# a-rtemis99/hpc_suffix_array

Hardware: AMD Instinct MI355X
Metric: suffixes sorted/sec + ms/doubling-round, 1 GiB input at 1/2/4/8 MI355X (higher is better)
Workload: dtype u32

## Files before the change

### hpc_suffix_array_amd/_native.py

```python
from __future__ import annotations

import ctypes
import os
import subprocess

PKG_DIR = os.path.dirname(os.path.abspath(__file__))
LIB_PATH = os.path.join(PKG_DIR, "lib", "libsa_hip.so")
LIB_PATH = os.environ.get("SA_LIB_PATH", LIB_PATH)
CSRC = os.path.join(PKG_DIR, "csrc")

SA_MAX_ROUNDS = 64
KERNEL_KINDS = ["init", "hist_first", "hist_keys", "scan", "scatter_first", "scatter_keys",
                "heads", "heads_scan", "rerank", "seg_count", "seg_scan", "seg_write", "alphabet", "pack",
                "sort_u", "windows", "local_sort", "pivot_keys", "pivot_count", "pivot_write"]
SCHEDULE_PACKED = 0
SCHEDULE_REFERENCE = 1
ROUND1_AUTO = 0
ROUND1_LSD = 1
ROUND1_BUCKETED = 2
SA_K_COUNT = len(KERNEL_KINDS)
FIND_AUTO = 0
FIND_LANE = 1
FIND_WAVE = 2
FIND_LANE_MAX = 3584
# ... 41 lines not shown
EXT_SYMBOLS = ["sa_context_create", "sa_context_destroy", "sa_context_set_debug", "sa_workspace_bytes", "sa_build_device",
               "sa_build_ex", "sa_check_device", "sa_check", "sa_lcp_device", "sa_lcp", "sa_generate_text_device",
               "sa_alphabet_device", "sa_pack_keys_device", "sa_sort_pairs_device", "sa_scatter_u64_device",
               "sa_gather_u64_device", "sa_running_max_i64_device", "sa_inclusive_sum_i64_device",
               "sa_count_below_u64_device", "sa_select_u8_device",
               "sa_find_device", "sa_find", "sa_find_ex",
               "sa_match_device", "sa_matching_stats_device", "sa_match", "sa_matching_stats",
               "sa_bwt_device", "sa_bwt", "sa_inverse_device", "sa_inverse",
               "sa_locate_device", "sa_locate",
               "sa_mems_device", "sa_mems",
               "sa_lpf_device", "sa_lpf", "sa_lz77_device", "sa_lz77",
               "sa_repeats_device", "sa_repeats",
               "sa_lf_device", "sa_ibwt_device", "sa_lf", "sa_ibwt", "sa_ibwt_ex",
               "sa_fm_index_bytes", "sa_fm_build_device", "sa_fm_count_device", "sa_fm_locate_device",
               "sa_fm_build", "sa_fm_count", "sa_fm_locate",
               "sa_doc_array_device", "sa_doc_of_device", "sa_doc_frequency_device", "sa_doc_list_device",
               "sa_doc_array", "sa_doc_of", "sa_doc_frequency", "sa_doc_list",
               "sa_lce_index_bytes", "sa_lce_build_device", "sa_lcp_min_device", "sa_lce_device",
               "sa_substr_compare_device", "sa_lcp_min", "sa_lce", "sa_substr_compare",
               "sa_dist_begin", "sa_dist_cuts", "sa_dist_plan_cuts", "sa_dist_reserve", "sa_dist_release", "sa_dist_round1", "sa_dist_req_count", "sa_dist_req_fill",
               "sa_dist_answer", "sa_dist_refine",
               "sa_last_error", "sa_host_syncs", "sa_device_count", "sa_version", "sa_struct_size"]


class SAError(RuntimeError):
    """A libsa_hip entry point returned an error code."""


DEBUG_FLAGS = {"no_cmp": 0x1, "no_pk8": 0x2, "no_pad": 0x4, "pad_overflow": 0x8, "no_fast32": 0x10,
               "no_pivot": 0x20, "perm_always": 0x40, "no_xq": 0x80, "xq_overflow": 0x100,
               "no_tied": 0x200, "no_key1_round": 0x400, "no_eonly": 0x800,
               "eonly": 0x1000, "fast32_small": 0x2000, "no_round2_fused": 0x4000,
               "ls_one_wg": 0x8000, "no_alpha_sample": 0x10000, "alpha_sample_small": 0x20000,
               "bb17": 0x40000, "bb18": 0x80000}


def debug_bits(names) -> int:
    bits = 0
    for x in names or ():
        if x not in DEBUG_FLAGS:
            raise ValueError(f"unknown debug flag {x!r} (one of {sorted(DEBUG_FLAGS)})")
        bits |= DEBUG_FLAGS[x]
    return bits


class SaOpts(ctypes.Structure):
    _fields_ = [("profile", ctypes.c_int32), ("schedule", ctypes.c_int32), ("init_chars", ctypes.c_int32),
                ("radix", ctypes.c_int32), ("round1", ctypes.c_int32), ("debug", ctypes.c_uint32),
                ("span_extra", ctypes.c_int32), ("tune", ctypes.c_int32)]


class SaStats(ctypes.Structure):
    _fields_ = [
        ("rounds", ctypes.c_int32),
        ("n_kinds", ctypes.c_int32),
        ("total_ms", ctypes.c_double),
        ("h2d_ms", ctypes.c_double),
        ("d2h_ms", ctypes.c_double),
        ("round_ms", ctypes.c_double * SA_MAX_ROUNDS),
        ("distinct", ctypes.c_uint64 * SA_MAX_ROUNDS),
        ("passes", ctypes.c_int32 * SA_MAX_ROUNDS),
        ("sorted_n", ctypes.c_uint64 * SA_MAX_ROUNDS),
        ("prefix_len", ctypes.c_uint64 * SA_MAX_ROUNDS),
        ("schedule", ctypes.c_int32),
        ("init_chars", ctypes.c_int32),
        ("sigma", ctypes.c_int32),
        ("sparse_ranks", ctypes.c_int32),
# ... 290 lines not shown
```

### hpc_suffix_array_amd/csrc/sa_bucket.h

```cpp
#pragma once
#include <type_traits>

#include "sa_kernels.h"

namespace sa {

#ifndef SA_BS_BLOCK
#define SA_BS_BLOCK 512
#endif
constexpr int kBsBlock = SA_BS_BLOCK;
#ifndef SA_BS_ITEMS
#define SA_BS_ITEMS 18
#endif
constexpr int kBsItems = SA_BS_ITEMS;
constexpr int kBsCap = kBsBlock * kBsItems;
constexpr uint32_t kWinStride = 1024;
#ifndef SA_BS_WPC
#define SA_BS_WPC 2
#endif
constexpr uint32_t kBsWpc = SA_BS_WPC;
#ifndef SA_BS_GRID
#define SA_BS_GRID (1u << 22)
#endif
constexpr uint32_t kBsGrid = SA_BS_GRID;
constexpr uint64_t kBucketMinN = 1ull << 20;
constexpr uint32_t kLoBits = 8;
constexpr uint32_t kLoRadix = 1u << kLoBits;

__device__ __forceinline__ uint32_t bucket_of(uint64_t key1, uint32_t rb, uint64_t cmul, uint32_t bsh) {
    return (uint32_t)(((key1 >> rb) * cmul) >> bsh);
}

__device__ __forceinline__ uint32_t bucket_dmin(uint32_t b, uint64_t cmul, uint32_t bsh) {
    const uint64_t d0 = ((uint64_t)b << bsh) / cmul;
    return (uint32_t)((((d0 * cmul) >> bsh) == b) ? d0 : d0 + 1);
}
// ... 1271 lines not shown
                    }
                }
            }
        }
        probe.mark(5);
        store_window<BLOCK, ITEMS>(s_w, a, m, ib, mn, keys_out, sa_out, so.ksh);
        __syncthreads();
        probe.mark(6);
    }
    probe.flush(words);
    flush_totals(words, th, tu, tg);
}

template <int ITEMS>
__device__ __forceinline__ uint32_t slot0() {
    uint32_t t = threadIdx.x;
    asm volatile("" : "+v"(t));
    return (t / kWave) * (kWave * ITEMS) + (t & (kWave - 1));
}

constexpr uint32_t kSlotBits = kBsCap > (1 << 14) ? 15 : 14;
constexpr uint32_t kSlotMask = (1u << kSlotBits) - 1u;
constexpr uint32_t kLowMax = 32 - kSlotBits;
static_assert(kBsCap <= (1 << kSlotBits), "load slots in kSlotBits");
constexpr int kHdrWord = 14;
constexpr int kTicketWord = 15;

__global__ __launch_bounds__(kBlock) void k_window_split(const uint32_t* __restrict__ list,
                                                         const uint32_t* __restrict__ ws, BucketRel br,
                                                         uint32_t* __restrict__ words, uint4* __restrict__ hdr,
                                                         uint32_t* __restrict__ retry, uint32_t fast,
                                                         const uint32_t* __restrict__ pc = nullptr,
                                                         const uint32_t* __restrict__ pn = nullptr, uint32_t nb = 0,
                                                         uint32_t* __restrict__ hx = nullptr, uint32_t crows = 0) {
    const uint32_t nlist = words[7];
    const uint32_t lane = lane_id();
    for (uint64_t q0 = (uint64_t)blockIdx.x * kBlock; q0 < nlist; q0 += (uint64_t)gridDim.x * kBlock) {
        const uint64_t q = q0 + threadIdx.x;
        uint32_t j = 0, b0 = 0;
        bool one = false;
        const bool ok = q < nlist;
        if (ok) {
            j = list[q];
            b0 = br.wb[j];
            one = fast && br.wb[j + 1] - b0 == 1u;
            if (one && hx) {
                uint32_t nr = 0;
                for (uint32_t k = 0; k < kXq; ++k) {
                    const uint32_t c = pn[(uint64_t)k * nb + b0];
                    if (!crows && c && c < kWave) one = false;
                    nr += (c + kWave - 1) / kWave;
                }
                if (crows && nr > crows) one = false;
            }
        }
        const uint64_t m1 = __ballot(ok && one), m2 = __ballot(ok && !one);
        uint32_t base1 = 0, base2 = 0;
        if (lane == 0) {
            if (m1) base1 = atomicAdd(&words[kHdrWord], (uint32_t)__popcll(m1));
            if (m2) base2 = atomicAdd(&words[kRetryWord], (uint32_t)__popcll(m2));
        }
        base1 = (uint32_t)__shfl((int)base1, 0, kWave);
        base2 = (uint32_t)__shfl((int)base2, 0, kWave);
        if (ok && one) {
            const uint32_t a = ws[j];
            const uint32_t qi = base1 + (uint32_t)__popcll(m1 & lanemask_lt());
            hdr[qi] = make_uint4(j, a, ws[j + 1] - a, br.bdmin[b0]);
            if (hx) {
                uint32_t P = 0;
                for (uint32_t k = 0; k < kXq; ++k) {
                    const uint32_t c = pc[(uint64_t)k * nb + b0];
                    hx[(uint64_t)qi * 16 + k] = c - P;
                    if (k) hx[(uint64_t)qi * 16 + kXq - 1 + k] = P;
                    P += pn[(uint64_t)k * nb + b0];
                }
            }
        } else if (ok) {
            retry[base2 + (uint32_t)__popcll(m2 & lanemask_lt())] = j;
        }
    }
}

__global__ __launch_bounds__(kBlock) void k_window_gather(const uint32_t* __restrict__ list,
                                                          const uint32_t* __restrict__ words,
                                                          const uint32_t* __restrict__ ws,
                                                          const uint32_t* __restrict__ wb,
                                                          const uint32_t* __restrict__ pc,
                                                          const uint32_t* __restrict__ pn, uint32_t nb,
                                                          const uint64_t* __restrict__ in,
                                                          uint64_t* __restrict__ out) {
    const uint32_t nlist = words[kRetryWord];
    for (uint32_t qi = blockIdx.x; qi < nlist; qi += gridDim.x) {
        const uint32_t j = list[qi];
        uint64_t dst = ws[j];
        for (uint32_t b = wb[j]; b < wb[j + 1]; ++b) {
            for (uint32_t k = 0; k < kXq; ++k) {
                const uint32_t c = pn[(uint64_t)k * nb + b];
                const uint64_t src = pc[(uint64_t)k * nb + b];
                for (uint32_t t = threadIdx.x; t < c; t += kBlock) out[dst + t] = in[src + t];
                dst += c;
            }
        }
    }
}

template <int N, int LSV = 0>
__device__ __forceinline__ bool sort_sub_words(uint32_t* __restrict__ s_k, const uint32_t* __restrict__ s_x,
// ... 38 lines not shown
        const uint32_t x = s_k[k];
        uint32_t y = k;
        while (y > lo && s_k[y - 1] > x) {
            s_k[y] = s_k[y - 1];
            --y;
        }
        s_k[y] = x;
    }
    uint32_t pr = ~0u, cur = s_k[lo] >> kSlotBits;
    for (uint32_t k = lo; k < hi; ++k) {
        const uint32_t nx = k + 1 < hi ? (s_k[k + 1] >> kSlotBits) : ~0u;
        const bool eqp = k > lo && pr == cur, eqn = k + 1 < hi && nx == cur;
        nu += (eqp || eqn) ? 1u : 0u;
        ng += (!eqp && eqn) ? 1u : 0u;
        pr = cur;
        cur = nx;
    }
}

template <int ITEMS, int I0 = 0, int I1 = ITEMS>
__device__ __forceinline__ void load_items(const uint64_t* __restrict__ w_in, uint64_t a, uint32_t m,
                                           uint64_t (&x)[ITEMS]) {
    const uint32_t l0 = slot0<ITEMS>();
#pragma unroll
    for (int i = I0; i < I1; ++i) {
        const uint32_t le = l0 + i * kWave;
        x[i] = w_in[a + (le < m ? le : m - 1)];
    }
}

struct XqWin {
    const uint32_t* __restrict__ hx = nullptr;
    const uint32_t* __restrict__ rows = nullptr;
};

__device__ __forceinline__ uint32_t xq_offset(const uint32_t* __restrict__ hx, uint32_t le) {
    uint32_t off = hx[0];
#pragma unroll
    for (int k = 1; k < (int)kXq; ++k) off = hx[kXq - 1 + k] <= le ? hx[k] : off;
    return off;
}

template <int ITEMS, int I0 = 0, int I1 = ITEMS>
__device__ __forceinline__ void load_items_cr(const uint64_t* __restrict__ w_in, const uint32_t (&rv)[3],
                                              uint64_t (&x)[ITEMS]) {
    const uint32_t lane = lane_id();
#pragma unroll
    for (int i = I0; i < I1; ++i) {
        const uint32_t base = (uint32_t)__builtin_amdgcn_readlane((int)rv[0], i);
        x[i] = (w_in + base)[lane];
    }
}

template <int ITEMS, int ROWS>
__device__ __forceinline__ void load_rows_xq(const uint32_t* __restrict__ rows, uint32_t (&rv)[3]) {
    const uint32_t lane = lane_id();
    const uint32_t w = (uint32_t)__builtin_amdgcn_readfirstlane((int)(threadIdx.x / kWave));
    const uint32_t r = w * ITEMS + (lane < (uint32_t)ITEMS ? lane : 0u);
#pragma unroll
    for (int t = 0; t < 3; ++t) rv[t] = rows[t * ROWS + r];
}

template <int ITEMS, int I0 = 0, int I1 = ITEMS>
__device__ __forceinline__ void load_items_xq(const uint64_t* __restrict__ w_in, const uint32_t (&rv)[3], uint32_t m,
                                              uint64_t (&x)[ITEMS]) {
    const uint32_t l0 = slot0<ITEMS>();
    const uint32_t lane = lane_id();
    const uint32_t last = m - 1;
#pragma unroll
    for (int i = I0; i < I1; ++i) {
        const uint32_t le = l0 + i * kWave;
        const uint32_t lc = le < m ? le : last;
        const uint32_t da = (uint32_t)__builtin_amdgcn_readlane((int)rv[0], i);
        const uint32_t db = (uint32_t)__builtin_amdgcn_readlane((int)rv[1], i);
        const uint32_t sp = (uint32_t)__builtin_amdgcn_readlane((int)rv[2], i);
        x[i] = w_in[(uint32_t)((lane < sp ? da : db) + lc)];
    }
}

template <bool CR>
__global__ __launch_bounds__(kBlock) void k_window_rows(const uint32_t* __restrict__ words, const uint4* __restrict__ hdr,
                                                        const uint32_t* __restrict__ hx, uint32_t nrows,
                                                        uint32_t* __restrict__ rows) {
    const uint32_t nh = words[kHdrWord];
    const uint32_t lane = lane_id();
    for (uint64_t q = (uint64_t)blockIdx.x * kWaves + wave_id(); q < nh; q += (uint64_t)gridDim.x * kWaves) {
        const uint32_t m = hdr[q].z;
        uint32_t hv[16];
#pragma unroll
        for (int k = 0; k < 16; ++k) hv[k] = hx[q * 16 + k];
        if constexpr (CR) {
            uint32_t st[kXq], cn[kXq], nfull = 0;
#pragma unroll
            for (int k = 0; k < (int)kXq; ++k) {
                const uint32_t p0 = k ? hv[kXq - 1 + k] : 0u, p1 = k + 1 < (int)kXq ? hv[kXq + k] : m;
                st[k] = hv[k] + p0;
                cn[k] = p1 - p0;
                nfull += cn[k] / kWave;
            }
            for (uint32_t r = lane; r < nrows; r += kWave) {
                uint32_t base = st[0], cnt = 0, rf = 0, rp = nfull;
#pragma unroll
                for (int k = 0; k < (int)kXq; ++k) {
                    const uint32_t nf = cn[k] / kWave, rem = cn[k] % kWave;
                    if (r >= rf && r < rf + nf) {
                        base = st[k] + kWave * (r - rf);
                        cnt = kWave;
                    }
                    if (rem && r == rp) {
                        base = st[k] + kWave * nf;
                        cnt = rem;
                    }
                    rf += nf;
                    rp += rem ? 1u : 0u;
                }
                uint32_t* const e = rows + q * 3 * nrows + r;
                e[0] = base;
                e[nrows] = cnt;
            }
            continue;
        }
        for (uint32_t r = lane; r < nrows; r += kWave) {
            const uint32_t lo = std::min(r * kWave, m - 1), hi = std::min(r * kWave + (kWave - 1), m - 1);
            uint32_t split = kWave;
#pragma unroll
            for (int k = kXq - 1; k >= 1; --k) {
                const uint32_t pk = hv[kXq - 1 + k];
                if (pk > lo && pk <= hi) split = pk - r * kWave;
            }
            uint32_t* const e = rows + q * 3 * nrows + r;
            e[0] = xq_offset(hv, lo);
            e[nrows] = xq_offset(hv, hi);
            e[2 * nrows] = split;
        }
    }
}

#ifndef SA_LS_WFULL
#define SA_LS_WFULL 1
#endif
#ifndef SA_LS_CLAIMS
#define SA_LS_CLAIMS 1
#endif
#ifndef SA_LS_HRANK
#define SA_LS_HRANK 1
#endif
#ifndef SA_LS_HRANK_PF
#define SA_LS_HRANK_PF 3
#endif
#if SA_LS_HRANK_PF == 0
#define SA_LS_PF_TABLE {0, 0, 18, 18, 18}
#elif SA_LS_HRANK_PF == 1
#define SA_LS_PF_TABLE {18, 18, 18, 18, 18}
#elif SA_LS_HRANK_PF == 3
#define SA_LS_PF_TABLE {6, 6, 12, 18, 18}
#elif SA_LS_HRANK_PF == 5
#define SA_LS_PF_TABLE {0, 0, 6, 12, 18}
#elif SA_LS_HRANK_PF == 6
#define SA_LS_PF_TABLE {3, 6, 9, 15, 18}
#endif
constexpr int kLsPfHr[5] = SA_LS_PF_TABLE;
constexpr int kLsPfOld[5] = {0, 0, 18, 18, 18};
template <int P>
using pf_point = std::integral_constant<int, P>;
template <int BLOCK, int ITEMS, class Probe = NoProbe, bool XQ = false, int LSV = 0, bool CR = false>
__global__ __launch_bounds__(BLOCK, 4) void k_bucket_sort(const uint64_t* __restrict__ keys_in,
                                                       const uint4* __restrict__ hdr, uint32_t rb, uint32_t bits,
                                                       uint32_t ib, uint32_t* __restrict__ words,
                                                       uint64_t* __restrict__ keys_out, uint32_t* __restrict__ sa_out,
                                                       uint32_t* __restrict__ retry, SegOut so, XqWin xw = XqWin{}) {
    constexpr int WAVES = BLOCK / kWave;
    constexpr int CAP = BLOCK * ITEMS;
    static_assert(CAP <= (1 << kSlotBits), "load slots");
    __shared__ uint32_t s_lds[kSubBuckets / 2 + CAP + ((LSV & 1) ? kNet : 0) + CAP];
    uint32_t* const s_cnt = s_lds;
    uint32_t* const s_k = s_lds + kSubBuckets / 2;
    uint32_t* const s_x = s_k + CAP + ((LSV & 1) ? kNet : 0);
    __shared__ uint32_t s_tmp[WAVES];
    __shared__ uint32_t s_cm[WAVES];
    __shared__ uint32_t s_ug[WAVES];
    __shared__ uint32_t s_q[2];
    __shared__ unsigned long long s_tot[3];
    constexpr int WPT = kSubBuckets / 2 / BLOCK;
    static_assert(WPT * 2 == 4 && WPT * 2 * BLOCK == kSubBuckets, "four sub-buckets per thread");
    constexpr int ROWS = WAVES * ITEMS;

    const uint32_t wave = wave_id(), lane = lane_id();
    const uint32_t dg = threadIdx.x;
    const uint32_t nwin = words[kHdrWord];
    const uint32_t low_bits = bits - kSubBits;
    const uint32_t dsh = ib + low_bits;
    const uint32_t lmask = (1u << low_bits) - 1u;
    const uint64_t imask = (1ull << ib) - 1ull;
    auto end_of = [&](uint32_t sb) -> uint32_t { return ((s_cnt[sb >> 1] >> (16 * (sb & 1))) & 0xFFFFu) >> 2; };
    static_assert(4 * CAP < (1 << 16), "byte counts in 16-bit halves");
    auto cnt_word = [&](uint32_t y) -> uint32_t* {
        return reinterpret_cast<uint32_t*>(reinterpret_cast<char*>(s_cnt) + ((y << 1) & 0xFFCu));
    };
    auto half_inc = [](uint32_t y) -> uint32_t {
        uint32_t r;
        asm("v_lshlrev_b32_e64 %0, %1, 4" : "=v"(r) : "v"(y << 4));
        return r;
    };
    constexpr bool HR = SA_LS_HRANK != 0;
    typedef uint16_t __attribute__((may_alias)) half_t;
    Probe probe;
    if (threadIdx.x == 0) {
        s_q[0] = atomicAdd(&words[kTicketWord], 1u);
        if constexpr (HR) s_q[1] = atomicAdd(&words[kTicketWord], 1u);
        s_tot[0] = s_tot[1] = s_tot[2] = 0;
    }
    if constexpr (HR)
        for (int i = threadIdx.x; i < kSubBuckets / 2; i += BLOCK) s_cnt[i] = 0;
    __syncthreads();
    uint32_t q = (uint32_t)__builtin_amdgcn_readfirstlane((int)s_q[0]);
    if (q >= nwin) return;
    uint4 h = hdr[q];
    uint64_t w[ITEMS];
    uint32_t rv[3] = {0u, 0u, 0u};
    if constexpr (XQ) {
        load_rows_xq<ITEMS, ROWS>(xw.rows + (uint64_t)q * 3 * ROWS, rv);
        if constexpr (CR) load_items_cr<ITEMS>(keys_in, rv, w);
        else load_items_xq<ITEMS>(keys_in, rv, h.z, w);
    } else {
        load_items<ITEMS>(keys_in, h.y, h.z, w);
    }
    uint32_t qn = 0;
    bool more = false;
    uint4 hn = make_uint4(0u, 0u, 1u, 0u);
    uint32_t rwn[3] = {0u, 0u, 0u};
    auto next_window = [&](uint32_t ticket, uint32_t cur, uint32_t& qx, bool& mx, uint4& hx,
                           uint32_t (&rx)[3]) __attribute__((always_inline)) {
        qx = (uint32_t)__builtin_amdgcn_readfirstlane((int)ticket);
        mx = qx < nwin;
        hx = make_uint4(0u, 0u, 1u, 0u);
        if (mx) hx = hdr[qx];
        if constexpr (XQ) load_rows_xq<ITEMS, ROWS>(xw.rows + (uint64_t)(mx ? qx : cur) * 3 * ROWS, rx);
    };
    if constexpr (HR) next_window(s_q[1], q, qn, more, hn, rwn);
    uint32_t par = 0;
    for (;;) {
        probe.mark(-1);
        const uint32_t j = h.x, m = h.z;
        const uint64_t a = h.y;
        const uint64_t mn = (uint64_t)h.w << rb;
        if constexpr (!HR) {
            if (threadIdx.x == 0) s_q[par ^ 1u] = atomicAdd(&words[kTicketWord], 1u);
            for (int i = threadIdx.x; i < kSubBuckets / 2; i += BLOCK) s_cnt[i] = 0;
            __syncthreads();
            next_window(s_q[par ^ 1u], q, qn, more, hn, rwn);
        }
        probe.mark(0);
        const uint32_t l0 = slot0<ITEMS>();
        const bool wfull = SA_LS_WFULL && (wave + 1) * (uint32_t)(kWave * ITEMS) <= m;
        bool sfull = wfull;
        if constexpr (XQ && CR)
            sfull = SA_LS_WFULL && __ballot(lane < (uint32_t)ITEMS && rv[1] == kWave) == (1ull << ITEMS) - 1ull;
        auto slot_ok = [&](int i) -> bool {
            if constexpr (XQ && CR) return lane < (uint32_t)__builtin_amdgcn_readlane((int)rv[1], i);
            else return l0 + i * kWave < m;
        };
        static_assert(ITEMS == 18, "SA_LS_PF_TABLE");
        auto prefetch_at = [&](auto pc, auto rest) __attribute__((always_inline)) {
            constexpr int P = decltype(pc)::value;
            constexpr int A = P ? (HR ? kLsPfHr[P - 1] : kLsPfOld[P - 1]) : 0;
            constexpr int B = decltype(rest)::value ? ITEMS : (HR ? kLsPfHr[P] : kLsPfOld[P]);
            if constexpr (A < B) {
                __builtin_amdgcn_sched_barrier(0);
                if constexpr (XQ && CR) load_items_cr<ITEMS, A, B>(keys_in, rwn, w);
                else if constexpr (XQ) load_items_xq<ITEMS, A, B>(keys_in, rwn, hn.z, w);
                else load_items<ITEMS, A, B>(keys_in, hn.y, hn.z, w);
            }
        };
        constexpr std::false_type part{};
        constexpr std::true_type rest{};
        constexpr int RKW = (ITEMS + 3) / 4;
        uint32_t kk[HR ? ITEMS : 1], rk[HR ? RKW : 1];
        uint32_t tk = 0;
        static_assert(4 * kMaxSub <= 256, "byte ranks in 8 bits");
        if constexpr (HR) {
#pragma unroll
            for (int r = 0; r < RKW; ++r) rk[r] = 0;
            auto count1 = [&](int i, uint32_t le) {
                const uint32_t k = (uint32_t)(w[i] >> ib);
                const uint32_t y = k >> low_bits;
                const uint32_t old = atomicAdd(cnt_word(y), half_inc(y));
                s_x[le] = (uint32_t)(w[i] & imask);
                kk[i] = k;
                rk[i / 4] |= __builtin_amdgcn_ubfe(old, y << 4, 8u) << (8 * (i % 4));
            };
            if (sfull) {
#pragma unroll
                for (int i = 0; i < ITEMS; ++i) count1(i, l0 + i * kWave);
            } else {
#pragma unroll
                for (int i = 0; i < ITEMS; ++i) {
                    kk[i] = 0;
                    if (slot_ok(i)) count1(i, l0 + i * kWave);
                }
            }
            __builtin_amdgcn_sched_barrier(0);
// ... 427 lines not shown
```

### hpc_suffix_array_amd/csrc/sa_round1.h

```cpp
#pragma once

#ifndef SA_HIST_WPC
#define SA_HIST_WPC 64
#endif
#ifndef SA_REC_STRIPED
#define SA_REC_STRIPED 1
#endif
#ifndef SA_BB_EXTRA
#define SA_BB_EXTRA 0
#endif
#ifndef SA_ITEMS_A
#define SA_ITEMS_A 12
#endif
#ifndef SA_TEXT_BLOCK
#define SA_TEXT_BLOCK 512
#endif
#ifndef SA_LIST_BLOCK
#define SA_LIST_BLOCK 1024
#endif


#ifndef SA_SEG_BLOCK
#define SA_SEG_BLOCK 1024
#endif
// ... 463 lines not shown
        hipLaunchKernelGGL(k_bucket_starts<R>, dim3(gb), dim3(kBlock), 0, s, (const uint32_t*)(padded ? dlo : os_base(c)), \
                           hbase, (const uint32_t*)c->segw, m, bp.bs.cmul, bp.bs.bsh, bstart, bdmin, blo)
        switch (hb) {
            case 7: SA_BSTARTS(128); break;
            case 8: SA_BSTARTS(256); break;
            case 9: SA_BSTARTS(512); break;
            default: SA_BSTARTS(1024); break;
        }
#undef SA_BSTARTS
    }
    tm.end();
    add_bytes(st, SA_K_SCATTER_KEYS, (pk8 ? 16 : 20) * m);
    SA_HIP(hipGetLastError());
    const uint64_t nw = (m + kWinStride - 1) / kWinStride;
    uint32_t* ws = c->vals_alt;
    uint32_t* list = c->vals_alt + nw + 1;
    tm.begin(SA_K_WINDOWS);
    {
        const uint32_t g1 = (uint32_t)std::min<uint64_t>((nw + kBlock) / kBlock, 8192);
        hipLaunchKernelGGL(k_window_starts_tab, dim3(g1), dim3(kBlock), 0, s, (const uint32_t*)(c->segw + kBstartOff),
                           nb_tab, m, nw, ws, list + 4 * nw + 2);
        const uint32_t g2 = (uint32_t)std::min<uint64_t>((nw + kBlock - 1) / kBlock, 1024);
        hipLaunchKernelGGL(k_window_list, dim3(g2), dim3(kBlock), 0, s, (const uint32_t*)ws, nw, list, c->words);
    }
    tm.end();
    add_bytes(st, SA_K_WINDOWS, 8 * nw);
    SA_HIP(hipGetLastError());
    SA_HIP(hipMemcpyAsync(c->host_words, c->words, 48, hipMemcpyDeviceToHost, s));
    uint32_t* skew = list + nw;
    uint32_t* cnt_u = skew + nw;
    uint32_t* cnt_g = cnt_u + nw + 1;
    uint32_t* const rank_arr = br_.rank ? br_.rank : c->rank;
    uint32_t* const member = br_.member ? br_.member : c->member;
    SA_HIP(hipEventRecord(c->ev[kSyncEv], s));
    SA_HIP(hipMemsetAsync(cnt_u, 0, (2 * nw + 2) * 4, s));
    SA_HIP(hipMemsetAsync(member, 0, (n + 31) / 32 * 4, s));
    SA_HIP(host_sync_event(c->ev[kSyncEv]));
    if (c->alpha_prove && c->host_words[kAlphaBadWord]) {
        c->alpha_refuted = true;
        return SA_OK;
    }
    if (c->host_words[4]) return set_err(SA_E_INTERNAL, "radix look-back did not complete");
    if (padded && c->host_words[11]) {
        SA_TRACE("  bucketed round 1: padded segment overflow, again with exact digit totals");
        const int rc = round1_bucketed(c, d_text, n, d_sa, bp, br_, s, tm, st, done, fused, seg, ksh, false, allow_xq,
                                       round2);
        if (st) st->round1_segments = 2;
        return rc;
    }
    if (xq && c->host_words[9]) {
        SA_TRACE("  bucketed round 1: second-pass queue overflow, again with one region");
        return round1_bucketed(c, d_text, n, d_sa, bp, br_, s, tm, st, done, fused, seg, ksh, allow_pad, false,
                               round2);
    }
    if (st) st->largest_window = (int32_t)std::min<uint32_t>(c->host_words[5], INT32_MAX);
    if (c->host_words[5] > (uint32_t)kBsCap) {
        SA_TRACE("  bucketed round 1: window of %u > %d suffixes, full sort instead", c->host_words[5], kBsCap);
        return SA_OK;
    }
    BucketRel br{cnt_g + nw + 1, c->segw + kBstartOff, c->segw + kBstartOff + kBstartWords, bp.bs.rb};
    br.bits1 = bits1;
    SegOut so{rank_arr, member, br_.sa_off, c->u_pos[1], c->u_idx[1], c->u_g[1], cnt_u, cnt_g, kKeySample};
    so.tmp_rank = br_.prefix ? br_.tmp_rank : nullptr;
    so.samples = (SA_LAZY_SAMPLES && !br_.always_u && !(c->dbg & SA_DEBUG_NO_KEY1_ROUND)) ? 0u : 1u;
    uint32_t* const retry = cnt_g + 2 * nw + 2;
    BucketRel br_measured = br;
    br_measured.bits1 = 0;
    uint4* const hdr = reinterpret_cast<uint4*>(((uintptr_t)(retry + nw + 4) + 15) & ~(uintptr_t)15);
    uint32_t* const hx = xq ? reinterpret_cast<uint32_t*>(hdr + nw + 1) : nullptr;
    constexpr uint32_t kBsRows = (kBsBlock / kWave) * kBsItems;
    uint32_t* const xrows = xq ? hx + 16 * (nw + 1) : nullptr;
    const uint64_t* const wide_in = xq ? c->keys[1] : c->keys_u;
    auto local_sort = [&](const SegOut& o) {
        const uint32_t g = std::max<uint32_t>(1, std::min(c->host_words[7], kBsGrid));
        static_assert(kRetryWord == kUsFlagWord + 1, "one memset clears words[12..15]");
        (void)hipMemsetAsync(c->words + kUsFlagWord, 0, 16, s);
        if (fast32) {
            const uint32_t gs = (uint32_t)std::max<uint64_t>(1, std::min<uint64_t>((nw + kBlock - 1) / kBlock, 1024));
            const bool cr = xq && !(((uint32_t)c->tune >> 29) & 1u);
            const uint32_t ls_grid = (c->dbg & SA_DEBUG_LS_ONE_WG) ? 1u : kBsWpc * (uint32_t)c->cus;
            hipLaunchKernelGGL(k_window_split, dim3(gs), dim3(kBlock), 0, s, (const uint32_t*)list, (const uint32_t*)ws,
                               br, c->words, hdr, retry, 1u, (const uint32_t*)xq_pc, (const uint32_t*)xq_pn, nb_tab, hx,
                               cr ? kBsRows : 0u);
            if (xq) {
                if (cr)
                    hipLaunchKernelGGL(k_window_rows<true>, dim3(2048), dim3(kBlock), 0, s, (const uint32_t*)c->words,
                                       (const uint4*)hdr, (const uint32_t*)hx, kBsRows, xrows);
                else
                    hipLaunchKernelGGL(k_window_rows<false>, dim3(2048), dim3(kBlock), 0, s, (const uint32_t*)c->words,
                                       (const uint4*)hdr, (const uint32_t*)hx, kBsRows, xrows);
                XqWin xw;
                xw.hx = hx;
                xw.rows = xrows;
#define SA_LS_XQ(V, CR)                                                                                          \
    hipLaunchKernelGGL((k_bucket_sort<kBsBlock, kBsItems, NoProbe, true, V, CR>), dim3(ls_grid), dim3(kBsBlock), 0, \
                       s, (const uint64_t*)c->keys_u, (const uint4*)hdr, bp.bs.rb, br.bits1, bp.ib, c->words,      \
                       c->keys[0], d_sa, retry, o, xw)
                switch (ls_variant(c) | (cr ? 4 : 0)) {
                case 1: SA_LS_XQ(1, false); break;
                case 2: SA_LS_XQ(2, false); break;
                case 3: SA_LS_XQ(3, false); break;
                case 4: SA_LS_XQ(0, true); break;
                case 5: SA_LS_XQ(1, true); break;
                case 6: SA_LS_XQ(2, true); break;
                case 7: SA_LS_XQ(3, true); break;
                default: SA_LS_XQ(0, false); break;
                }
#undef SA_LS_XQ
                hipLaunchKernelGGL(k_window_gather, dim3(1024), dim3(kBlock), 0, s, (const uint32_t*)retry,
                                   (const uint32_t*)c->words, (const uint32_t*)ws, (const uint32_t*)br.wb,
                                   (const uint32_t*)xq_pc, (const uint32_t*)xq_pn, nb_tab, (const uint64_t*)c->keys_u,
                                   c->keys[1]);
            } else {
#define SA_LS(V)                                                                                                 \
    hipLaunchKernelGGL((k_bucket_sort<kBsBlock, kBsItems, NoProbe, false, V>), dim3(ls_grid), dim3(kBsBlock), 0, \
                       s, (const uint64_t*)c->keys_u, (const uint4*)hdr, bp.bs.rb, br.bits1, bp.ib, c->words,   \
                       c->keys[0], d_sa, retry, o)
                switch (ls_variant(c)) {
                case 1: SA_LS(1); break;
                case 2: SA_LS(2); break;
                case 3: SA_LS(3); break;
                default: SA_LS(0); break;
                }
#undef SA_LS
            }
        } else {
            hipLaunchKernelGGL((k_bucket_sort_wide<kBsBlock, kBsItems>), dim3(g), dim3(kBsBlock), 0, s,
                               (const uint64_t*)c->keys_u, br, (const uint32_t*)ws, (const uint32_t*)list, c->words,
                               bp.ib, c->keys[0], d_sa, skew, o, br.bits1 ? retry : (uint32_t*)nullptr, 7u);
        }
        if (br.bits1)
            hipLaunchKernelGGL((k_bucket_sort_wide<kBsBlock, kBsItems>), dim3(std::min<uint32_t>(g, 1024)),
                               dim3(kBsBlock), 0, s, wide_in, br_measured, (const uint32_t*)ws,
                               (const uint32_t*)retry, c->words, bp.ib, c->keys[0], d_sa, skew, o, (uint32_t*)nullptr,
                               (uint32_t)kRetryWord);
        const uint32_t gl = std::min<uint32_t>(g, 1024);
        hipLaunchKernelGGL((k_bucket_sort_lsd<kBsBlock, kBsItems>), dim3(gl), dim3(kBsBlock), 0, s,
                           wide_in, br, (const uint32_t*)ws, (const uint32_t*)skew, c->words, bp.ib,
                           c->keys[0], d_sa, o);
    };
    tm.begin(SA_K_LOCAL_SORT);
    local_sort(so);
    tm.end();
    add_bytes(st, SA_K_LOCAL_SORT, 12 * m + (so.samples ? (m >> kKeySample) * 8 : 0));
    SA_HIP(hipGetLastError());
    auto gather_u = [&]() {
        const uint32_t wb = (uint32_t)((nw + 1 + kWsBlock - 1) / kWsBlock);
        uint32_t* part = c->hist;
        hipLaunchKernelGGL(k_wscan_reduce, dim3(wb), dim3(kBlock), 0, s, (const uint32_t*)cnt_u, (const uint32_t*)cnt_g,
                           nw, part);
        hipLaunchKernelGGL(k_wscan_top, dim3(1), dim3(kBlock), 0, s, part, wb);
        hipLaunchKernelGGL(k_wscan_apply, dim3(wb), dim3(kBlock), 0, s, cnt_u, cnt_g, nw, (const uint32_t*)part);
        const uint32_t g = (uint32_t)std::max<uint64_t>(1, std::min<uint64_t>((c->host_words[7] + kWaves - 1) / kWaves, 4096));
        RankMap rm;
        if (br_.prefix) {
            const uint64_t nwb = (n + 31) / 32;
            const uint32_t pb = (uint32_t)((nwb + kPcBlock - 1) / kPcBlock);
            uint32_t* ppart = br_.prefix + nwb + 1;
            hipLaunchKernelGGL(k_popc_reduce, dim3(pb), dim3(kBlock), 0, s, (const uint32_t*)member, nwb, ppart);
            hipLaunchKernelGGL(k_popc_top, dim3(1), dim3(kPcTop), 0, s, ppart, pb);
            hipLaunchKernelGGL(k_popc_apply, dim3(pb), dim3(kBlock), 0, s, (const uint32_t*)member, nwb,
                               (const uint32_t*)ppart, br_.prefix);
            rm = RankMap{member, br_.prefix};
        }
        hipLaunchKernelGGL(k_u_gather, dim3(g), dim3(kBlock), 0, s, (const uint32_t*)list, (const uint32_t*)c->words,
                           (const uint32_t*)ws, (const uint32_t*)cnt_u, (const uint32_t*)cnt_g, so, c->u_pos[0],
                           c->u_idx[0], c->u_g[0], rm);
    };
    const bool try_r2 = round2 && so.rank && !br_.always_u && !so.tmp_rank && br_.sa_off == 0 &&
                        !(c->dbg & (SA_DEBUG_NO_KEY1_ROUND | SA_DEBUG_NO_ROUND2_FUSED)) && key1_bits(bp.bs) <= 64;
    if (try_r2) {
        tm.round_mark();
        tm.begin(SA_K_SORT_U);
        const uint64_t per = (uint64_t)kWaves * kR2Batch;
        const uint32_t g = (uint32_t)std::max<uint64_t>(1, std::min<uint64_t>((c->host_words[7] + per - 1) / per, 65536));
// ... 17 lines not shown
    if (c->host_words[6]) {
        SA_TRACE("  bucketed round 1: local sort flags %u, full sort instead", c->host_words[6]);
        if (try_r2) tm.round_unmark();
        return SA_OK;
    }
    seg[0] = c->host_words[0];
    seg[1] = c->host_words[1];
    seg[2] = c->host_words[2];
    add_bytes(st, SA_K_LOCAL_SORT, seg[1] * 28);
    const bool sparse = br_.always_u || seg[1] <= n / kSparseDiv;
    if (try_r2) {
        add_bytes(st, SA_K_SORT_U, seg[1] * 28);
        if (!sparse) {
            tm.round_unmark();
        } else if (c->host_words[kUsFlagWord] == 0) {
            SA_TRACE("  bucketed round 1: round 2 finished from the staging (%llu members)",
                     (unsigned long long)seg[1]);
            *round2 = 2;
        } else {
            SA_TRACE("  bucketed round 1: round 2 from the staging gave up, the set compacted");
            *round2 = 1;
            tm.begin(SA_K_SEG_WRITE);
            gather_u();
            tm.end();
            SA_HIP(hipGetLastError());
        }
    }
    if (!try_r2 || *round2 == 1) add_bytes(st, SA_K_SEG_WRITE, 8 * (2 * nw + 2) + seg[1] * 24);
    if (!sparse) {
        SegOut full{};
        full.ksh = 0;
        SA_HIP(hipMemsetAsync(c->words + 10, 0, 4, s));
        tm.begin(SA_K_LOCAL_SORT);
        local_sort(full);
        tm.end();
        add_bytes(st, SA_K_LOCAL_SORT, 20 * m);
        SA_HIP(hipGetLastError());
    } else {
        *ksh = kKeySample;
        *fused = true;
        c->samples_pending = so.samples == 0u;
    }
    SA_TRACE("  bucketed round 1: s=%u R=%u rb=%u cmp=%u pk8=%d windows=%u (skewed %u) largest=%u", bp.bs.s, bp.bs.R,
             bp.bs.rb, bp.bs.cmp, pk8 ? 1 : 0, c->host_words[7], c->host_words[10], c->host_words[5]);
    *done = true;
    return SA_OK;
}
```

### include/sa_hip.h

```cpp
#ifndef SA_HIP_H
#define SA_HIP_H

#include <stdint.h>

#ifdef __cplusplus
extern "C" {
#endif

#define SA_OK 0
#define SA_E_INVALID (-1)
#define SA_E_NOMEM (-2)
#define SA_E_HIP (-3)
#define SA_E_INTERNAL (-4)

#define SA_MAX_ROUNDS 64

enum sa_kernel_kind {
    SA_K_INIT = 0,
    SA_K_HIST_FIRST = 1,
    SA_K_HIST_KEYS = 2,
    SA_K_SCAN = 3,
    SA_K_SCATTER_FIRST = 4,
    SA_K_SCATTER_KEYS = 5,
    SA_K_HEADS = 6,
// ... 11 lines not shown
    SA_K_PIVOT_COUNT = 18,
    SA_K_PIVOT_WRITE = 19,
    SA_K_COUNT = 20
};

#define SA_ROUND1_AUTO 0
#define SA_ROUND1_LSD 1
#define SA_ROUND1_BUCKETED 2
#define SA_ROUND1_PIVOT 3

#define SA_SCHEDULE_PACKED 0
#define SA_SCHEDULE_REFERENCE 1

#define SA_DEBUG_NO_CMP 0x1u
#define SA_DEBUG_NO_PK8 0x2u
#define SA_DEBUG_NO_PAD 0x4u
#define SA_DEBUG_PAD_OVERFLOW 0x8u
#define SA_DEBUG_NO_FAST32 0x10u
#define SA_DEBUG_NO_PIVOT 0x20u
#define SA_DEBUG_PERM_ALWAYS 0x40u
#define SA_DEBUG_NO_XQ 0x80u
#define SA_DEBUG_XQ_OVERFLOW 0x100u
#define SA_DEBUG_NO_KEY1_ROUND 0x400u
#define SA_DEBUG_NO_TIED 0x200u
#define SA_DEBUG_NO_EONLY 0x800u
#define SA_DEBUG_EONLY 0x1000u
#define SA_DEBUG_FAST32_SMALL 0x2000u
#define SA_DEBUG_NO_ROUND2_FUSED 0x4000u
#define SA_DEBUG_LS_ONE_WG 0x8000u
#define SA_DEBUG_NO_ALPHA_SAMPLE 0x10000u
#define SA_DEBUG_ALPHA_SAMPLE_SMALL 0x20000u
#define SA_DEBUG_BB17 0x40000u
#define SA_DEBUG_BB18 0x80000u

#define SA_ALPHABET_EXACT 0
#define SA_ALPHABET_SAMPLED 1
#define SA_ALPHABET_REFUTED 2

typedef struct {
    int32_t profile;
    int32_t schedule;
    int32_t init_chars;
    int32_t radix;
    int32_t round1;
    uint32_t debug;
    int32_t span_extra;
    int32_t tune;
} sa_opts;

typedef struct {
    int32_t rounds;
    int32_t n_kinds;
    double total_ms;
    double h2d_ms, d2h_ms;
    double round_ms[SA_MAX_ROUNDS];
    uint64_t distinct[SA_MAX_ROUNDS];
    int32_t passes[SA_MAX_ROUNDS];
    uint64_t sorted_n[SA_MAX_ROUNDS];
    uint64_t prefix_len[SA_MAX_ROUNDS];
    int32_t schedule;
    int32_t init_chars;
    int32_t sigma;
    int32_t sparse_ranks;
    int32_t round1;
    int32_t largest_window;
    uint64_t model_bytes;
// ... 271 lines not shown
```

Measured before the change: 112.7 billion.

## Pack per-window row descriptors and decode rows in-wave instead of row table

Replaces the per-window row table (3×ROWS words built by a separate k_window_rows kernel) with a 32-word packed chunk descriptor written by k_window_split. The bucket sort kernel loads one word per lane and reconstructs each row's base and count with readlane and ds_bpermute. This drops a kernel launch and cuts global traffic for row metadata. It also moves the window split ahead of the host sync so it overlaps with the host wait. The old row-table path stays behind a new debug flag.

New measurement: 112.2 billion. About the same (-0.4%).

```diff
diff --git a/hpc_suffix_array_amd/_native.py b/hpc_suffix_array_amd/_native.py
--- a/hpc_suffix_array_amd/_native.py
+++ b/hpc_suffix_array_amd/_native.py
@@ -97,7 +97,7 @@
                "no_tied": 0x200, "no_key1_round": 0x400, "no_eonly": 0x800,
                "eonly": 0x1000, "fast32_small": 0x2000, "no_round2_fused": 0x4000,
                "ls_one_wg": 0x8000, "no_alpha_sample": 0x10000, "alpha_sample_small": 0x20000,
-               "bb17": 0x40000, "bb18": 0x80000}
+               "bb17": 0x40000, "bb18": 0x80000, "row_table": 0x100000}
 
 
 def debug_bits(names) -> int:
diff --git a/hpc_suffix_array_amd/csrc/sa_bucket.h b/hpc_suffix_array_amd/csrc/sa_bucket.h
--- a/hpc_suffix_array_amd/csrc/sa_bucket.h
+++ b/hpc_suffix_array_amd/csrc/sa_bucket.h
@@ -2,6 +2,7 @@
 #include <type_traits>
 
 #include "sa_kernels.h"
+#include "sa_rows.h"
 
 namespace sa {
 
@@ -1339,7 +1340,8 @@
                                                          uint32_t* __restrict__ retry, uint32_t fast,
                                                          const uint32_t* __restrict__ pc = nullptr,
                                                          const uint32_t* __restrict__ pn = nullptr, uint32_t nb = 0,
-                                                         uint32_t* __restrict__ hx = nullptr, uint32_t crows = 0) {
+                                                         uint32_t* __restrict__ hx = nullptr, uint32_t crows = 0,
+                                                         uint32_t* __restrict__ pk = nullptr) {
     const uint32_t nlist = words[7];
     const uint32_t lane = lane_id();
     for (uint64_t q0 = (uint64_t)blockIdx.x * kBlock; q0 < nlist; q0 += (uint64_t)gridDim.x * kBlock) {
@@ -1374,12 +1376,20 @@
             const uint32_t qi = base1 + (uint32_t)__popcll(m1 & lanemask_lt());
             hdr[qi] = make_uint4(j, a, ws[j + 1] - a, br.bdmin[b0]);
             if (hx) {
-                uint32_t P = 0;
+                uint32_t hv[16], P = 0;
+#pragma unroll
                 for (uint32_t k = 0; k < kXq; ++k) {
                     const uint32_t c = pc[(uint64_t)k * nb + b0];
-                    hx[(uint64_t)qi * 16 + k] = c - P;
-                    if (k) hx[(uint64_t)qi * 16 + kXq - 1 + k] = P;
+                    hv[k] = c - P;
+                    if (k) hv[kXq - 1 + k] = P;
                     P += pn[(uint64_t)k * nb + b0];
+                }
+#pragma unroll
+                for (uint32_t k = 0; k < 2 * kXq - 1; ++k) hx[(uint64_t)qi * 16 + k] = hv[k];
+                if (pk) {
+                    uint32_t st[kXq], cn[kXq];
+                    chunk_bounds(hv, ws[j + 1] - a, st, cn);
+                    chunk_pack(st, cn, pk + (uint64_t)qi * kRowPackWords);
                 }
             }
         } else if (ok) {
@@ -1484,6 +1494,7 @@
 struct XqWin {
     const uint32_t* __restrict__ hx = nullptr;
     const uint32_t* __restrict__ rows = nullptr;
+    const uint32_t* __restrict__ pk = nullptr;
 };
 
 __device__ __forceinline__ uint32_t xq_offset(const uint32_t* __restrict__ hx, uint32_t le) {
@@ -1511,6 +1522,28 @@
     const uint32_t r = w * ITEMS + (lane < (uint32_t)ITEMS ? lane : 0u);
 #pragma unroll
     for (int t = 0; t < 3; ++t) rv[t] = rows[t * ROWS + r];
+}
+
+__device__ __forceinline__ uint32_t load_pack_xq(const uint32_t* __restrict__ pk32) {
+    return pk32[lane_id() & (kRowPackWords - 1u)];
+}
+
+struct PackLanes {
+    uint32_t w;
+    __device__ __forceinline__ uint32_t u(uint32_t i) const {
+        return (uint32_t)__builtin_amdgcn_readlane((int)w, (int)i);
+    }
+    __device__ __forceinline__ uint32_t v(uint32_t i) const {
+        return (uint32_t)__builtin_amdgcn_ds_bpermute((int)(i << 2), (int)w);
+    }
+};
+
+template <int ITEMS>
+__device__ __forceinline__ void rows_from_pack(uint32_t (&rv)[3]) {
+    static_assert(kXq == kRowChunks && (uint32_t)kWave == kRowSlots, "sa_rows.h");
+    const uint32_t lane = lane_id();
+    const uint32_t w = (uint32_t)__builtin_amdgcn_readfirstlane((int)(threadIdx.x / kWave));
+    chunk_row_packed(PackLanes{rv[2]}, w * ITEMS + (lane < (uint32_t)ITEMS ? lane : 0u), rv[0], rv[1]);
 }
 
 template <int ITEMS, int I0 = 0, int I1 = ITEMS>
@@ -1542,30 +1575,11 @@
 #pragma unroll
         for (int k = 0; k < 16; ++k) hv[k] = hx[q * 16 + k];
         if constexpr (CR) {
-            uint32_t st[kXq], cn[kXq], nfull = 0;
-#pragma unroll
-            for (int k = 0; k < (int)kXq; ++k) {
-                const uint32_t p0 = k ? hv[kXq - 1 + k] : 0u, p1 = k + 1 < (int)kXq ? hv[kXq + k] : m;
-                st[k] = hv[k] + p0;
-                cn[k] = p1 - p0;
-                nfull += cn[k] / kWave;
-            }
+            uint32_t st[kXq], cn[kXq];
+            chunk_bounds(hv, m, st, cn);
             for (uint32_t r = lane; r < nrows; r += kWave) {
-                uint32_t base = st[0], cnt = 0, rf = 0, rp = nfull;
-#pragma unroll
-                for (int k = 0; k < (int)kXq; ++k) {
-                    const uint32_t nf = cn[k] / kWave, rem = cn[k] % kWave;
-                    if (r >= rf && r < rf + nf) {
-                        base = st[k] + kWave * (r - rf);
-                        cnt = kWave;
-                    }
-                    if (rem && r == rp) {
-                        base = st[k] + kWave * nf;
-                        cnt = rem;
-                    }
-                    rf += nf;
-                    rp += rem ? 1u : 0u;
-                }
+                uint32_t base, cnt;
+                chunk_row(st, cn, r, base, cnt);
                 uint32_t* const e = rows + q * 3 * nrows + r;
                 e[0] = base;
                 e[nrows] = cnt;
@@ -1615,7 +1629,7 @@
 constexpr int kLsPfOld[5] = {0, 0, 18, 18, 18};
 template <int P>
 using pf_point = std::integral_constant<int, P>;
-template <int BLOCK, int ITEMS, class Probe = NoProbe, bool XQ = false, int LSV = 0, bool CR = false>
+template <int BLOCK, int ITEMS, class Probe = NoProbe, bool XQ = false, int LSV = 0, bool CR = false, bool RT = false>
 __global__ __launch_bounds__(BLOCK, 4) void k_bucket_sort(const uint64_t* __restrict__ keys_in,
                                                        const uint4* __restrict__ hdr, uint32_t rb, uint32_t bits,
                                                        uint32_t ib, uint32_t* __restrict__ words,
@@ -1670,7 +1684,12 @@
     uint4 h = hdr[q];
     uint64_t w[ITEMS];
     uint32_t rv[3] = {0u, 0u, 0u};
-    if constexpr (XQ) {
+    constexpr bool HX = XQ && CR && !RT;
+    if constexpr (HX) {
+        rv[2] = load_pack_xq(xw.pk + (uint64_t)q * kRowPackWords);
+        rows_from_pack<ITEMS>(rv);
+        load_items_cr<ITEMS>(keys_in, rv, w);
+    } else if constexpr (XQ) {
         load_rows_xq<ITEMS, ROWS>(xw.rows + (uint64_t)q * 3 * ROWS, rv);
         if constexpr (CR) load_items_cr<ITEMS>(keys_in, rv, w);
         else load_items_xq<ITEMS>(keys_in, rv, h.z, w);
@@ -1687,7 +1706,8 @@
         mx = qx < nwin;
         hx = make_uint4(0u, 0u, 1u, 0u);
         if (mx) hx = hdr[qx];
-        if constexpr (XQ) load_rows_xq<ITEMS, ROWS>(xw.rows + (uint64_t)(mx ? qx : cur) * 3 * ROWS, rx);
+        if constexpr (HX) rx[2] = load_pack_xq(xw.pk + (uint64_t)(mx ? qx : cur) * kRowPackWords);
+        else if constexpr (XQ) load_rows_xq<ITEMS, ROWS>(xw.rows + (uint64_t)(mx ? qx : cur) * 3 * ROWS, rx);
     };
     if constexpr (HR) next_window(s_q[1], q, qn, more, hn, rwn);
     uint32_t par = 0;
@@ -1719,6 +1739,7 @@
             constexpr int B = decltype(rest)::value ? ITEMS : (HR ? kLsPfHr[P] : kLsPfOld[P]);
             if constexpr (A < B) {
                 __builtin_amdgcn_sched_barrier(0);
+                if constexpr (HX && A == 0) rows_from_pack<ITEMS>(rwn);
                 if constexpr (XQ && CR) load_items_cr<ITEMS, A, B>(keys_in, rwn, w);
                 else if constexpr (XQ) load_items_xq<ITEMS, A, B>(keys_in, rwn, hn.z, w);
                 else load_items<ITEMS, A, B>(keys_in, hn.y, hn.z, w);
diff --git a/hpc_suffix_array_amd/csrc/sa_round1.h b/hpc_suffix_array_amd/csrc/sa_round1.h
--- a/hpc_suffix_array_amd/csrc/sa_round1.h
+++ b/hpc_suffix_array_amd/csrc/sa_round1.h
@@ -519,9 +519,33 @@
     uint32_t* cnt_g = cnt_u + nw + 1;
     uint32_t* const rank_arr = br_.rank ? br_.rank : c->rank;
     uint32_t* const member = br_.member ? br_.member : c->member;
+    BucketRel br{cnt_g + nw + 1, c->segw + kBstartOff, c->segw + kBstartOff + kBstartWords, bp.bs.rb};
+    br.bits1 = bits1;
+    uint32_t* const retry = cnt_g + 2 * nw + 2;
+    uint4* const hdr = reinterpret_cast<uint4*>(((uintptr_t)(retry + nw + 4) + 15) & ~(uintptr_t)15);
+    uint32_t* const hx = xq ? reinterpret_cast<uint32_t*>(hdr + nw + 1) : nullptr;
+    constexpr uint32_t kBsRows = (kBsBlock / kWave) * kBsItems;
+    uint32_t* const xrows = xq ? hx + 16 * (nw + 1) : nullptr;
+    const bool cr = xq && !(((uint32_t)c->tune >> 29) & 1u);
+    const bool row_table = cr && (c->dbg & SA_DEBUG_ROW_TABLE);
+    uint32_t* const xpk = cr && !row_table ? xrows : nullptr;
+    auto window_split = [&]() {
+        static_assert(kRetryWord == kUsFlagWord + 1, "one memset clears words[12..15]");
+        (void)hipMemsetAsync(c->words + kUsFlagWord, 0, 16, s);
+        if (!fast32) return;
+        const uint32_t gs = (uint32_t)std::max<uint64_t>(1, std::min<uint64_t>((nw + kBlock - 1) / kBlock, 1024));
+        hipLaunchKernelGGL(k_window_split, dim3(gs), dim3(kBlock), 0, s, (const uint32_t*)list, (const uint32_t*)ws, br,
+                           c->words, hdr, retry, 1u, (const uint32_t*)xq_pc, (const uint32_t*)xq_pn, nb_tab, hx,
+                           cr ? kBsRows : 0u, xpk);
+    };
     SA_HIP(hipEventRecord(c->ev[kSyncEv], s));
     SA_HIP(hipMemsetAsync(cnt_u, 0, (2 * nw + 2) * 4, s));
     SA_HIP(hipMemsetAsync(member, 0, (n + 31) / 32 * 4, s));
+    if (fast32) {
+        tm.begin(SA_K_WINDOWS);
+        window_split();
+        tm.end();
+    }
     SA_HIP(host_sync_event(c->ev[kSyncEv]));
     if (c->alpha_prove && c->host_words[kAlphaBadWord]) {
         c->alpha_refuted = true;
@@ -545,53 +569,45 @@
         SA_TRACE("  bucketed round 1: window of %u > %d suffixes, full sort instead", c->host_words[5], kBsCap);
         return SA_OK;
     }
-    BucketRel br{cnt_g + nw + 1, c->segw + kBstartOff, c->segw + kBstartOff + kBstartWords, bp.bs.rb};
-    br.bits1 = bits1;
     SegOut so{rank_arr, member, br_.sa_off, c->u_pos[1], c->u_idx[1], c->u_g[1], cnt_u, cnt_g, kKeySample};
     so.tmp_rank = br_.prefix ? br_.tmp_rank : nullptr;
     so.samples = (SA_LAZY_SAMPLES && !br_.always_u && !(c->dbg & SA_DEBUG_NO_KEY1_ROUND)) ? 0u : 1u;
-    uint32_t* const retry = cnt_g + 2 * nw + 2;
     BucketRel br_measured = br;
     br_measured.bits1 = 0;
-    uint4* const hdr = reinterpret_cast<uint4*>(((uintptr_t)(retry + nw + 4) + 15) & ~(uintptr_t)15);
-    uint32_t* const hx = xq ? reinterpret_cast<uint32_t*>(hdr + nw + 1) : nullptr;
-    constexpr uint32_t kBsRows = (kBsBlock / kWave) * kBsItems;
-    uint32_t* const xrows = xq ? hx + 16 * (nw + 1) : nullptr;
     const uint64_t* const wide_in = xq ? c->keys[1] : c->keys_u;
-    auto local_sort = [&](const SegOut& o) {
+    auto local_sort = [&](const SegOut& o, bool split_done) {
         const uint32_t g = std::max<uint32_t>(1, std::min(c->host_words[7], kBsGrid));
-        static_assert(kRetryWord == kUsFlagWord + 1, "one memset clears words[12..15]");
-        (void)hipMemsetAsync(c->words + kUsFlagWord, 0, 16, s);
+        if (!split_done) window_split();
         if (fast32) {
-            const uint32_t gs = (uint32_t)std::max<uint64_t>(1, std::min<uint64_t>((nw + kBlock - 1) / kBlock, 1024));
-            const bool cr = xq && !(((uint32_t)c->tune >> 29) & 1u);
             const uint32_t ls_grid = (c->dbg & SA_DEBUG_LS_ONE_WG) ? 1u : kBsWpc * (uint32_t)c->cus;
-            hipLaunchKernelGGL(k_window_split, dim3(gs), dim3(kBlock), 0, s, (const uint32_t*)list, (const uint32_t*)ws,
-                               br, c->words, hdr, retry, 1u, (const uint32_t*)xq_pc, (const uint32_t*)xq_pn, nb_tab, hx,
-                               cr ? kBsRows : 0u);
             if (xq) {
-                if (cr)
+                if (row_table)
                     hipLaunchKernelGGL(k_window_rows<true>, dim3(2048), dim3(kBlock), 0, s, (const uint32_t*)c->words,
                                        (const uint4*)hdr, (const uint32_t*)hx, kBsRows, xrows);
-                else
+                else if (!cr)
                     hipLaunchKernelGGL(k_window_rows<false>, dim3(2048), dim3(kBlock), 0, s, (const uint32_t*)c->words,
                                        (const uint4*)hdr, (const uint32_t*)hx, kBsRows, xrows);
                 XqWin xw;
                 xw.hx = hx;
-                xw.rows = xrows;
-#define SA_LS_XQ(V, CR)                                                                                          \
-    hipLaunchKernelGGL((k_bucket_sort<kBsBlock, kBsItems, NoProbe, true, V, CR>), dim3(ls_grid), dim3(kBsBlock), 0, \
-                       s, (const uint64_t*)c->keys_u, (const uint4*)hdr, bp.bs.rb, br.bits1, bp.ib, c->words,      \
+                xw.rows = xpk ? nullptr : xrows;
+                xw.pk = xpk;
+#define SA_LS_XQ(V, CR, RT)                                                                                          \
+    hipLaunchKernelGGL((k_bucket_sort<kBsBlock, kBsItems, NoProbe, true, V, CR, RT>), dim3(ls_grid), dim3(kBsBlock), \
+                       0, s, (const uint64_t*)c->keys_u, (const uint4*)hdr, bp.bs.rb, br.bits1, bp.ib, c->words,      \
                        c->keys[0], d_sa, retry, o, xw)
-                switch (ls_variant(c) | (cr ? 4 : 0)) {
-                case 1: SA_LS_XQ(1, false); break;
-                case 2: SA_LS_XQ(2, false); break;
-                case 3: SA_LS_XQ(3, false); break;
-                case 4: SA_LS_XQ(0, true); break;
-                case 5: SA_LS_XQ(1, true); break;
-                case 6: SA_LS_XQ(2, true); break;
-                case 7: SA_LS_XQ(3, true); break;
-                default: SA_LS_XQ(0, false); break;
+                switch (ls_variant(c) | (cr ? 4 : 0) | (row_table ? 8 : 0)) {
+                case 1: SA_LS_XQ(1, false, false); break;
+                case 2: SA_LS_XQ(2, false, false); break;
+                case 3: SA_LS_XQ(3, false, false); break;
+                case 4: SA_LS_XQ(0, true, false); break;
+                case 5: SA_LS_XQ(1, true, false); break;
+                case 6: SA_LS_XQ(2, true, false); break;
+                case 7: SA_LS_XQ(3, true, false); break;
+                case 12: SA_LS_XQ(0, true, true); break;
+                case 13: SA_LS_XQ(1, true, true); break;
+                case 14: SA_LS_XQ(2, true, true); break;
+                case 15: SA_LS_XQ(3, true, true); break;
+                default: SA_LS_XQ(0, false, false); break;
                 }
 #undef SA_LS_XQ
                 hipLaunchKernelGGL(k_window_gather, dim3(1024), dim3(kBlock), 0, s, (const uint32_t*)retry,
@@ -627,7 +643,7 @@
                            c->keys[0], d_sa, o);
     };
     tm.begin(SA_K_LOCAL_SORT);
-    local_sort(so);
+    local_sort(so, fast32);
     tm.end();
     add_bytes(st, SA_K_LOCAL_SORT, 12 * m + (so.samples ? (m >> kKeySample) * 8 : 0));
     SA_HIP(hipGetLastError());
@@ -711,7 +727,7 @@
         full.ksh = 0;
         SA_HIP(hipMemsetAsync(c->words + 10, 0, 4, s));
         tm.begin(SA_K_LOCAL_SORT);
-        local_sort(full);
+        local_sort(full, false);
         tm.end();
         add_bytes(st, SA_K_LOCAL_SORT, 20 * m);
         SA_HIP(hipGetLastError());
diff --git a/hpc_suffix_array_amd/csrc/sa_rows.h b/hpc_suffix_array_amd/csrc/sa_rows.h
--- /dev/null
+++ b/hpc_suffix_array_amd/csrc/sa_rows.h
@@ -0,0 +1,93 @@
+#pragma once
+#include <stdint.h>
+
+#if defined(__HIPCC__) || defined(__HIP__)
+#define SA_HD __host__ __device__ __forceinline__
+#else
+#define SA_HD inline
+#endif
+
+namespace sa {
+
+constexpr uint32_t kRowChunks = 8;
+constexpr uint32_t kRowSlots = 64;
+
+template <class H>
+SA_HD void chunk_bounds(const H& hv, uint32_t m, uint32_t (&st)[kRowChunks], uint32_t (&cn)[kRowChunks]) {
+#if defined(__HIP_DEVICE_COMPILE__)
+#pragma unroll
+#endif
+    for (uint32_t k = 0; k < kRowChunks; ++k) {
+        const uint32_t p0 = k ? hv[kRowChunks - 1 + k] : 0u;
+        const uint32_t p1 = k + 1 < kRowChunks ? hv[kRowChunks + k] : m;
+        st[k] = hv[k] + p0;
+        cn[k] = p1 - p0;
+    }
+}
+
+SA_HD void chunk_row(const uint32_t (&st)[kRowChunks], const uint32_t (&cn)[kRowChunks], uint32_t r, uint32_t& base,
+                     uint32_t& count) {
+    uint32_t nfull = 0;
+#if defined(__HIP_DEVICE_COMPILE__)
+#pragma unroll
+#endif
+    for (uint32_t k = 0; k < kRowChunks; ++k) nfull += cn[k] / kRowSlots;
+    base = st[0];
+    count = 0;
+    uint32_t rf = 0, rp = nfull;
+#if defined(__HIP_DEVICE_COMPILE__)
+#pragma unroll
+#endif
+    for (uint32_t k = 0; k < kRowChunks; ++k) {
+        const uint32_t nf = cn[k] / kRowSlots, rem = cn[k] % kRowSlots;
+        if (r - rf < nf) {
+            base = st[k] + kRowSlots * (r - rf);
+            count = kRowSlots;
+        }
+        if (rem && r == rp) {
+            base = st[k] + kRowSlots * nf;
+            count = rem;
+        }
+        rf += nf;
+        rp += rem ? 1u : 0u;
+    }
+}
+
+constexpr uint32_t kRowPackWords = 32;
+
+SA_HD void chunk_pack(const uint32_t (&st)[kRowChunks], const uint32_t (&cn)[kRowChunks], uint32_t* pk) {
+    uint32_t rf = 0, np = 0;
+    for (uint32_t k = 0; k < kRowChunks; ++k) {
+        const uint32_t nf = cn[k] / kRowSlots, rem = cn[k] % kRowSlots;
+        pk[k] = st[k] - kRowSlots * rf;
+        rf += nf;
+        pk[kRowChunks + k] = rf;
+        if (rem) {
+            pk[2 * kRowChunks + np] = st[k] + kRowSlots * nf;
+            pk[3 * kRowChunks + np] = rem;
+            ++np;
+        }
+    }
+    for (; np < kRowChunks; ++np) {
+        pk[2 * kRowChunks + np] = st[0];
+        pk[3 * kRowChunks + np] = 0;
+    }
+}
+
+template <class PK>
+SA_HD void chunk_row_packed(const PK& pk, uint32_t r, uint32_t& base, uint32_t& count) {
+    uint32_t a = pk.u(0);
+#if defined(__HIP_DEVICE_COMPILE__)
+#pragma unroll
+#endif
+    for (uint32_t k = 1; k < kRowChunks; ++k) a = r >= pk.u(kRowChunks + k - 1) ? pk.u(k) : a;
+    const uint32_t nfull = pk.u(2 * kRowChunks - 1);
+    const uint32_t t = r - nfull;
+    const uint32_t ti = t < kRowChunks ? t : kRowChunks - 1;
+    const uint32_t b = pk.v(2 * kRowChunks + ti), rem = pk.v(3 * kRowChunks + ti);
+    const bool full = r < nfull, part = t < kRowChunks;
+    base = full ? a + kRowSlots * r : part ? b : pk.u(0);
+    count = full ? kRowSlots : part ? rem : 0u;
+}
+
+}
diff --git a/include/sa_hip.h b/include/sa_hip.h
--- a/include/sa_hip.h
+++ b/include/sa_hip.h
@@ -67,6 +67,7 @@
 #define SA_DEBUG_ALPHA_SAMPLE_SMALL 0x20000u
 #define SA_DEBUG_BB17 0x40000u
 #define SA_DEBUG_BB18 0x80000u
+#define SA_DEBUG_ROW_TABLE 0x100000u
 
 #define SA_ALPHABET_EXACT 0
 #define SA_ALPHABET_SAMPLED 1
```
